# NilanEkanayake/TiTok-Video

Measured on AMD Instinct MI355X. Metric: video clips/sec encode+decode (whole node), higher is better.
Workload: dtype bf16

## Files before the change

include/titok_hip.h:

```cpp
#ifndef TITOK_HIP_H
#define TITOK_HIP_H

#include <stdint.h>

#ifdef __cplusplus
extern "C" {
#endif

#define TTV_OK 0
#define TTV_ERR_INVALID 1
#define TTV_ERR_LAUNCH 2
#define TTV_ERR_UNSUPPORTED 3

#define TTV_BF16 0
#define TTV_F32 1

#define TTV_ENCODER 0
#define TTV_DECODER 1

#define TTV_MAX_FSQ 8
#define TTV_MAX_TOKEN 64
#define TTV_MAX_CLIPS_PER_LAUNCH 64

const char* ttv_error_string(void);
// ... 112 lines not shown
int ttv_quant_v_pv8(const void* qkvg, int ld, const int32_t* cu_seqlens, int n_seqs, int total_rows, int q_heads, int kv_heads, void* image,
                    void* stream);
int ttv_attention_pv8(const void* qkvg, int ld, void* out, int ldo, const int32_t* cu_seqlens, const int32_t* qblocks, int n_qblocks,
                      int q_heads, int kv_heads, int head_dim, int flags, const void* image, void* stream);

int ttv_rmsnorm_mx(const void* in, int in_dtype, int ld_in, void* out, int out_dtype, int ld_out, const float* gain, int rows, int width,
                   float eps, float* next_rstd, void* mx_q, void* mx_s, void* stream);
int ttv_attention_mxout(const void* qkvg, int ld, void* out_q, void* out_mx, int ld_mx, const int32_t* cu_seqlens, const int32_t* qblocks,
                        int n_qblocks, int q_heads, int kv_heads, void* stream);
int ttv_linear_fp8_mx_geglu_q(const void* xq, int ldx, const void* x_mx, const float* x_row_scale, const void* wq, int ldw, const void* w_mx,
                              const float* w_row_scale, void* hq, void* hq_mx, int M, int N, int K, void* stream);

int ttv_row_rstd(const void* x, int dtype, int ldx, float* rstd, int rows, int width, float eps, void* stream);
int ttv_linear_rowscale(const void* x, int ldx, const void* w, int ldw, const float* row_scale, int epilogue, const float* rope_cs, int d_model,
                        int gqa_dim, void* y, int ldy, int M, int N, int K, int dtype, void* stream);

int ttv_patch_gather(const void* const* clips, const int32_t* clip_desc, int clip0, int n_clips, int patch_t, int patch_h,
                     int patch_w, int channels, void* patches, int ld, int dtype, int max_patches_per_clip, void* stream);
int ttv_patch_embed_norm(const void* const* clips, const int32_t* clip_desc, const int32_t* patch_rows, const int32_t* row_seq, int n_clips,
                         int patch_t, int patch_h, int patch_w, int channels, const void* w, int ldw, const void* bias,
                         const float* mask_token, const float* gain, float eps, void* x, int ldx, int rows, int width, int dtype,
                         void* stream);
int ttv_patch_scatter(const void* patches, int ld, const int32_t* clip_desc, int clip0, int n_clips, int patch_t, int patch_h,
                      int patch_w, int channels, void* const* clips, int dtype, int max_patches_per_clip, void* stream);

typedef struct ttv_tower_dims {
  int32_t kind;
  int32_t dtype;
  int32_t width;
  int32_t layers;
// ... 505 lines not shown
```

titok_video_amd/_lib.py:

```python
from __future__ import annotations

import ctypes as C
import os
import threading

import torch

from . import switches

TTV_BF16, TTV_F32 = 0, 1
TTV_ENCODER, TTV_DECODER = 0, 1
TTV_MAX_FSQ = 8
TTV_MAX_TOKEN = 64
TTV_MAX_CLIPS_PER_LAUNCH = 64
TTV_DISC_HEAD_GENERATOR, TTV_DISC_HEAD_DISCRIMINATOR = 0, 1
TTV_TAPE_STORED, TTV_TAPE_RECOMPUTE = 0, 1

DBG_NO_STORES = 1
DBG_K256_NO_PANEL_DMA = 2
DBG_MLP_NO_WEIGHT_DMA = 2
DBG_K256_NO_TILE_RELOAD = 4
DBG_MLP_NO_GEGLU = 4
DBG_K256_NO_EPILOGUE_MATH = 8
DBG_MLP_TILES8 = 8
# ... 211 lines not shown
    "ttv_layer_tail_fused": (C.c_int, [vp, C.c_int, vp, f32, vp, C.c_int, vp, C.c_int, vp, C.c_int, vp, f32, f32, C.c_int, C.c_int,
                                       C.c_int, vp, vp]),
    "ttv_mlp_fused": (C.c_int, [vp, C.c_int, vp, C.c_int, vp, C.c_int, vp, f32, f32, C.c_int, C.c_int, C.c_int, vp]),
    "ttv_fill_const_rows": (C.c_int, [vp, C.c_int, C.c_int, vp, C.c_int, C.c_int, vp, vp, f32, vp]),
    "ttv_decoder_embed": (C.c_int, [vp, C.c_int, vp, vp, vp, vp, vp, C.c_int, C.c_int, vp, C.c_int, C.c_int, f32, vp]),
    "ttv_attention": (C.c_int, [vp, C.c_int, vp, C.c_int, vp, vp, C.c_int, C.c_int, C.c_int, C.c_int, C.c_int, C.c_int, vp]),
    "ttv_attention64": (C.c_int, [vp, C.c_int, vp, C.c_int, vp, vp, C.c_int, C.c_int, C.c_int, C.c_int, C.c_int, C.c_int, vp]),
    "ttv_rmsnorm_mx": (C.c_int, [vp, C.c_int, C.c_int, vp, C.c_int, C.c_int, vp, C.c_int, C.c_int, f32, vp, vp, vp, vp]),
    "ttv_attention_pv8_bytes": (C.c_int64, [C.c_int, C.c_int, C.c_int]),
    "ttv_quant_v_pv8": (C.c_int, [vp, C.c_int, vp, C.c_int, C.c_int, C.c_int, C.c_int, vp, vp]),
    "ttv_attention_pv8": (C.c_int, [vp, C.c_int, vp, C.c_int, vp, vp, C.c_int, C.c_int, C.c_int, C.c_int, C.c_int, vp, vp]),
    "ttv_attention_mxout": (C.c_int, [vp, C.c_int, vp, vp, C.c_int, vp, vp, C.c_int, C.c_int, C.c_int, vp]),
    "ttv_linear_fp8_mx_geglu_q": (C.c_int, [vp, C.c_int, vp, vp, vp, C.c_int, vp, vp, vp, vp, C.c_int, C.c_int, C.c_int, vp]),
    "ttv_row_rstd": (C.c_int, [vp, C.c_int, C.c_int, vp, C.c_int, C.c_int, f32, vp]),
    "ttv_linear_rowscale": (C.c_int, [vp, C.c_int, vp, C.c_int, vp, C.c_int, vp, C.c_int, C.c_int, vp, C.c_int, C.c_int, C.c_int, C.c_int, C.c_int, vp]),
    "ttv_patch_gather": (C.c_int, [C.POINTER(vp), vp, C.c_int, C.c_int, C.c_int, C.c_int, C.c_int, C.c_int, vp, C.c_int,
                                   C.c_int, C.c_int, vp]),
    "ttv_patch_embed_norm": (C.c_int, [C.POINTER(vp), vp, vp, vp, C.c_int, C.c_int, C.c_int, C.c_int, C.c_int, vp, C.c_int, vp, vp, vp, f32,
                                       vp, C.c_int, C.c_int, C.c_int, C.c_int, vp]),
    "ttv_patch_scatter": (C.c_int, [vp, C.c_int, vp, C.c_int, C.c_int, C.c_int, C.c_int, C.c_int, C.c_int, C.POINTER(vp),
                                    C.c_int, C.c_int, vp]),
    "ttv_tower_workspace_bytes": (i64, [C.POINTER(TowerDims), C.POINTER(Batch)]),
    "ttv_encoder_forward": (C.c_int, [C.POINTER(TowerDims), C.POINTER(TowerWeights), C.POINTER(Batch), C.POINTER(vp),
                                      C.POINTER(FsqParams), vp, vp, vp, vp, vp, i64, vp]),
    "ttv_decoder_forward": (C.c_int, [C.POINTER(TowerDims), C.POINTER(TowerWeights), C.POINTER(Batch), vp, C.POINTER(vp),
                                      vp, i64, vp]),
    "ttv_dec_l0_const_bytes": (i64, [C.POINTER(TowerDims), C.c_int]),
    "ttv_dec_l0_const_build": (C.c_int, [C.POINTER(TowerDims), C.POINTER(TowerWeights), vp, vp, vp, vp, C.c_int, vp, i64, C.POINTER(i64), C.POINTER(i64), vp]),
    "ttv_decoder_forward_const": (C.c_int, [C.POINTER(TowerDims), C.POINTER(TowerWeights), C.POINTER(Batch), vp, C.POINTER(vp),
                                            vp, i64, C.POINTER(DecL0Const), vp]),
# ... 210 lines not shown
```

titok_video_amd/csrc/ttv_api.hip:

```cpp
#include <stdarg.h>
#include <stdio.h>
#include <stdlib.h>
#include <string.h>

#include "ttv_common.h"
#include "ttv_kernels.h"

static thread_local char g_err[512] = "";

void ttv_set_error(const char* fmt, ...) {
  va_list ap;
  va_start(ap, fmt);
  vsnprintf(g_err, sizeof(g_err), fmt, ap);
  va_end(ap);
}

int g_ttv_prof_class = 0;
bool ttv_sw_enc_latent_last() { static const bool v = ttv_env_flag("TTV_ENC_LATENT_LAST", true); return v; }
bool ttv_enc_latent_rows_only(const ttv_tower_dims* d, const ttv_batch* b) {
  return ttv_sw_enc_latent_last() && !(g_ttv_debug & TTV_DBG_ENC_ALL_ROWS) && d->kind == TTV_ENCODER && b->latent_rows && b->sum_tokens > 0 &&
         b->sum_tokens < b->total_rows;
}
bool ttv_sw_keel_f32sum() { static const bool v = ttv_env_flag("TTV_KEEL_F32SUM", false); return v; }
bool ttv_sw_fused_patch() { static const bool v = ttv_env_flag("TTV_FUSED_PATCH", true); return v; }
// ... 237 lines not shown
  const int nq = 2 * dm + 2 * g;
  const int64_t row_bytes = (int64_t)dm * dtype_bytes(dt);
  bool qkv_ready = false;
  bool rstd_valid = false;
  bool xq_valid = false;
  const bool lat_last = ttv_enc_latent_rows_only(d, b) && b->qblocks_latent && b->n_qblocks_latent > 0;
  static const bool pat_env = ttv_env_flag("TTV_DEC_PATCH_LAST", true);
  const bool pat_last = pat_env && !(g_ttv_debug & TTV_DBG_DEC_ALL_BLOCKS) && d->kind == TTV_DECODER && d->layers >= 2 && b->qblocks_patch &&
                        b->n_qblocks_patch > 0 && !split3 && !b->qblocks_paired;
  bool compacted = false;
  const bool pv8 = w->attn_pv8 != 0;
  TTV_CHECK_ARG(!pv8 || (dt == TTV_BF16 && !split3), "attn_pv8 is a bf16 inference option (not for fp32 or split-bf16 towers)");
  const LayerCtx ctx = {d, b, ws, s, split3, s3img, gen_ok, b->qblocks_paired ? TTV_ATTN_PAIRED : 0, b->qblocks_all_full ? TTV_ATTN_ALLFULL : 0,
                        ttv_sw_attn_pipe() ? TTV_ATTN_PIPE : 0, pv8};
  const bool l0_const = dec_l0_const_ok(ctx, w, l0);
  for (int i = 0; i < d->layers; ++i) {
    const ttv_layer_weights& lw = w->layers[i];
    const bool last = i == d->layers - 1;
    const bool l0c = l0_const && i == 0;
    if (dt == TTV_BF16 && dm != 256 && dm % 128 == 0 && d->inner % 128 == 0 && !ttv_sw_keel_f32sum() && lw.to_qkv_f8 && lw.to_qkv_mx && lw.w12_f8 &&
        lw.w12_mx && lw.out_proj_f8 && lw.out_proj_mx && lw.w3_f8 && lw.w3_mx &&
        !(lat_last && last)) {
      TTV_TRY(run_layer_mx(ctx, lw, i, rstd_valid, xq_valid));
      qkv_ready = false;
      continue;
    }
    xq_valid = false;
    const bool f8_qkv = rows_f8(dt, dm, lw.to_qkv_f8, lw.to_qkv_f8_scale, lw.to_qkv_mx, lw.to_qkv_pn);
    const bool f8_w12 = rows_f8(dt, dm, lw.w12_f8, lw.w12_f8_scale, lw.w12_mx, lw.w12_pn);
    if (!qkv_ready) {
      const void* w_plain = (dt == TTV_BF16 && lw.to_qkv_qs) ? lw.to_qkv_qs : lw.to_qkv;
      const PreNormW qw = {lw.pre_ln, w_plain, lw.to_qkv_pn, lw.to_qkv_f8, lw.to_qkv_f8_scale, f8_qkv};
      if (l0c) TTV_TRY(prenorm_proj(ctx, EPI_QKV_ROPE, ws.x, L, qw, nq, ws.qkv, 0, rstd_valid, l0->latent_rows / 128, (l0->latent_rows + l0->patch_rows) / 128));
      else if (lat_last && last && !f8_qkv && enc_last_qkv_skip_ok(ctx, lw))
        TTV_TRY(prenorm_proj(ctx, EPI_QKV_ROPE, ws.x, L, qw, nq, ws.qkv, 0, rstd_valid, b->tokens_per_clip / 128,
                             (b->tokens_per_clip + b->max_patches_per_clip) / 128, 2 * dm / 64));
      else TTV_TRY(prenorm_proj(ctx, EPI_QKV_ROPE, ws.x, L, qw, nq, ws.qkv, s3img ? 2 : 0, rstd_valid));
// ... 18 lines not shown
      TTV_TRY(tower_attention(ctx, q_scaled, b->qblocks, b->n_qblocks, ctx.pair | ctx.all_full | ctx.pipe));
    char* cx = ws.x;
    char* cao = ws.ao;
    int Lc = L;
    if (lat_now) {
      TTV_TRY(gather_rows(ws.x, ws.xl, b->latent_rows, b->sum_tokens, row_bytes, s));
      TTV_TRY(gather_rows(ws.ao, ws.aol, b->latent_rows, b->sum_tokens, row_bytes, s));
      cx = ws.xl; cao = ws.aol; Lc = b->sum_tokens;
      compacted = true;
    }
    static const bool use_fused_mlp = ttv_env_flag("TTV_FUSED_MLP", true);
    static const bool use_fused_qkv = ttv_env_flag("TTV_FUSED_QKV", false);
    const float alpha = keel_alpha(d, i);
    if (use_fused_mlp && ttvk_mlp_fused_supported(dt, dm, d->inner) && lw.mlp_pack) {
      MlpNextQkv nx = {};
      const bool back = use_fused_qkv && !last && lw.mlp_pack_qkv_rows == nq && nq % 64 == 0 && dm % 64 == 0 && g % 64 == 0;
      if (back) { nx.qkv = ws.qkv; nx.ld = nq; nx.rope_cs = b->rope_cs; nx.rows = nq; nx.rope_q_end = dm; nx.rope_k_begin = 2 * dm; nx.rope_k_end = 2 * dm + g; }
      TTV_TRY(ttvk_mlp_fused(cao, dm, i == 0 ? nullptr : lw.attn_post_ln, alpha, cx, dm, lw.mlp_pack, d->inner, cx, dm, i == 0 ? nullptr : lw.ffd_post_ln,
                             alpha, d->eps, Lc, back ? &nx : nullptr, s));
      qkv_ready = back;
      continue;
    }
    TTV_TRY(keel_tail(ctx, gemm_args(dt, cao, dm, lw.out_proj, dm, Lc, dm, dm, cx, dm), i, lw.attn_post_ln, gen_ok && lw.w12_pn && !f8_w12, rstd_valid));
    const PreNormW fw = {lw.ffd_norm, lw.w12, lw.w12_pn, lw.w12_f8, lw.w12_f8_scale, f8_w12};
    TTV_TRY(prenorm_proj(ctx, EPI_GEGLU, cx, Lc, fw, d->inner, ws.h, s3img, rstd_valid));
    rstd_valid = false;
    const ttv_layer_weights* nl = last ? nullptr : &w->layers[i + 1];
    const bool next_rstd = gen_ok && nl && nl->to_qkv_pn && !rows_f8(dt, dm, nl->to_qkv_f8, nl->to_qkv_f8_scale, nl->to_qkv_mx, nl->to_qkv_pn);
    TTV_TRY(keel_tail(ctx, gemm_args(dt, ws.h, d->inner, lw.w3, d->inner, Lc, dm, d->inner, cx, dm), i, lw.ffd_post_ln, next_rstd, rstd_valid));
  }
  if (compacted)
// ... 306 lines not shown
  TTV_CHECK_ARG(ldx >= width, "row_rstd: leading dim smaller than the width");
  return ttvk_row_rstd(x, dtype, ldx, rstd, rows, width, eps, (hipStream_t)stream);
}

int ttv_linear_rowscale(const void* x, int ldx, const void* w, int ldw, const float* row_scale, int epilogue, const float* rope_cs, int d_model,
                        int gqa_dim, void* y, int ldy, int M, int N, int K, int dtype, void* stream) {
  TTV_CHECK_ARG(M == 0 || (x && w && y), "linear_rowscale: null buffer");
  TTV_CHECK_ARG(epilogue >= 0 && epilogue <= 2, "linear_rowscale: epilogue 0 (store), 1 (qkv + rotary) or 2 (GEGLU)");
  GemmArgs a = gemm_args(dtype, x, ldx, w, ldw, M, N, K, y, ldy);
  if (epilogue == 1) {
    TTV_CHECK_ARG(rope_cs && N == 2 * d_model + 2 * gqa_dim && K == d_model, "linear_rowscale: qkv epilogue needs rope_cs, N = 2 d_model + 2 gqa_dim and K = d_model");
    a = gemm_rope_qk(a, rope_cs, d_model, gqa_dim);
  }
  a.row_scale = row_scale;
  return ttvk_gemm(epilogue == 0 ? EPI_STORE : epilogue == 1 ? EPI_QKV_ROPE : EPI_GEGLU, a, (hipStream_t)stream);
}

int ttv_patch_gather(const void* const* clips, const int32_t* clip_desc, int clip0, int n_clips, int patch_t, int patch_h, int patch_w,
                     int channels, void* patches, int ld, int dtype, int max_patches_per_clip, void* stream) {
  TTV_CHECK_ARG(n_clips == 0 || (clips && clip_desc && patches), "patch_gather: null buffer");
  return ttvk_patch_copy(false, (void* const*)clips, clip_desc, clip0, n_clips, patch_t, patch_h, patch_w, channels, patches, ld, dtype, max_patches_per_clip, (hipStream_t)stream);
}

int ttv_patch_embed_norm(const void* const* clips, const int32_t* clip_desc, const int32_t* patch_rows, const int32_t* row_seq, int n_clips,
                         int patch_t, int patch_h, int patch_w, int channels, const void* w, int ldw, const void* bias, const float* mask_token,
                         const float* gain, float eps, void* x, int ldx, int rows, int width, int dtype, void* stream) {
  TTV_CHECK_ARG(rows == 0 || (clips && clip_desc && patch_rows && row_seq && w && bias && mask_token && gain && x), "patch_embed_norm: null buffer");
  const int pd = channels * patch_t * patch_h * patch_w;
  if (!ttvk_patch_embed_norm_supported(dtype, width, pd, patch_w)) {
    ttv_set_error("patch_embed_norm: only bf16, width 256, patch_w 8 and a patch vector that is a multiple of 64");
// ... 411 lines not shown
```

titok_video_amd/csrc/ttv_mlp.hip:

```cpp
#include "ttv_common.h"
#include "ttv_kernels.h"

#define MLP_W12_CHUNKS 2048
#define MLP_W3_CHUNKS 1024
#define MLP_PANEL_CHUNKS (MLP_W12_CHUNKS + MLP_W3_CHUNKS)
#define MLP_WO_CHUNKS (4 * MLP_W12_CHUNKS)

struct MlpDev {
  const bf16_t* x; int ldx;
  const uint4* pack;
  const bf16_t* ao; int ldao;
  const float* front_gain;
  float front_alpha;
  bf16_t* qkv; int ldq;
  const float* rope_cs;
  int nqp, rope_q_end, rope_k_begin, rope_k_end;
  int I;
  bf16_t* y; int ldy;
  const float* post_gain;
  float alpha, eps;
  int M, n_tiles, debug;
  long long* stamps;
};

__global__ void k_mlp_pack(const bf16_t* __restrict__ w12f, const bf16_t* __restrict__ w3, const bf16_t* __restrict__ wo,
                           const bf16_t* __restrict__ wq, int nq_rows, int I, uint4* __restrict__ out) {
  const int np = I / 32;
  const int nqp = (nq_rows + 63) / 64;
  const int o = blockIdx.x * blockDim.x + threadIdx.x;
  if (o >= np * MLP_PANEL_CHUNKS + MLP_WO_CHUNKS + nqp * MLP_W12_CHUNKS) return;
  if (o >= np * MLP_PANEL_CHUNKS + MLP_WO_CHUNKS) {
    const int c = o - np * MLP_PANEL_CHUNKS - MLP_WO_CHUNKS, qp = c / MLP_W12_CHUNKS, cc = c - qp * MLP_W12_CHUNKS;
    const int r = cc >> 5, cp = cc & 31;
    const int ch = (cp & 16) | ((cp & 15) ^ (r & 15));
    int srow = qp * 64 + r;
    srow = srow < nq_rows ? srow : nq_rows - 1;
    const bf16_t* src = wq + (size_t)srow * 256 + (ch >> 2) * 32 + (ch & 3) * 4;
    const uint2 lo = *reinterpret_cast<const uint2*>(src), hi = *reinterpret_cast<const uint2*>(src + 16);
    out[o] = make_uint4(lo.x, lo.y, hi.x, hi.y);
    return;
  }
  if (o >= np * MLP_PANEL_CHUNKS) {
    const int c = o - np * MLP_PANEL_CHUNKS, wp = c / MLP_W12_CHUNKS, cc = c - wp * MLP_W12_CHUNKS;
    const int r = cc >> 5, cp = cc & 31;
    const int ch = (cp & 16) | ((cp & 15) ^ (r & 15));
    out[o] = wo ? *reinterpret_cast<const uint4*>(wo + (size_t)(wp * 64 + r) * 256 + ch * 8) : make_uint4(0, 0, 0, 0);
    return;
  }
  const int pn = o / MLP_PANEL_CHUNKS, c = o - pn * MLP_PANEL_CHUNKS;
  if (c < MLP_W12_CHUNKS) {
    const int r = c >> 5, cp = c & 31;
    const int ch = (cp & 16) | ((cp & 15) ^ (r & 15));
    const int srow = r < 32 ? pn * 32 + r : I + pn * 32 + (r - 32);
    const bf16_t* src = w12f + (size_t)srow * 256 + (ch >> 2) * 32 + (ch & 3) * 4;
// ... 24 lines not shown
                 "s_mov_b32 m0, %0"                                                                                \
                 : "=&s"(keep__)                                                                                   \
                 : "v"(lane16), "v"(lane16 + 8192u), "v"(lane16 + 16384u), "v"(lane16 + 24576u), "s"(src_), "s"(dst_) \
                 : "memory", "scc");                                                                               \
  } while (0)
#define MLP_GLDS_2(src_, dst_)                                                                                     \
  do {                                                                                                             \
    unsigned keep__;                                                                                               \
    asm volatile("s_mov_b32 %0, m0\n\t"                                                                            \
                 "s_mov_b32 m0, %4\n\ts_nop 0\n\tglobal_load_lds_dwordx4 %1, %3\n\t"                               \
                 "s_add_u32 m0, %4, 0x2000\n\ts_nop 0\n\tglobal_load_lds_dwordx4 %2, %3\n\t"                       \
                 "s_mov_b32 m0, %0"                                                                                \
                 : "=&s"(keep__)                                                                                   \
                 : "v"(lane16), "v"(lane16 + 8192u), "s"(src_), "s"(dst_)                                          \
                 : "memory", "scc");                                                                               \
  } while (0)
#ifdef MLP_STAMPS
#define MLP_STAMP()                                                                                                \
  do {                                                                                                             \
    if (p.stamps && blockIdx.x == 0 && (wave & 3) == 0 && lane == 0 && n_stamp < 64)                               \
      p.stamps[(wave >> 2) * 64 + n_stamp++] = (long long)__builtin_readcyclecounter();                            \
  } while (0)
#else
#define MLP_STAMP() do { (void)n_stamp; } while (0)
#endif

template <int TPB, int T1, int T2, bool GELU_FIRST, bool KEEL, bool FRONT, bool BACK>
__device__ __forceinline__ void mlp_wave(const MlpDev& p, uint4* l12, uint4* l3, uint4* hb, const float* gl, int tile, int wave, int lane,
                                         int P1F, int P2F, int& n_stamp) {
  constexpr int T1A = T1 > 0 ? T1 : 1, T2A = T2 > 0 ? T2 : 1;
// ... 250 lines not shown
  #pragma unroll
          for (int j = 0; j < T2; ++j) out[m][j] = __builtin_amdgcn_mfma_f32_16x16x32_bf16(w3f[m & 3], hf[j], out[m][j], 0, 0, 0);
          if (m + 4 < 16) w3f[m & 3] = __builtin_bit_cast(bf16x8, w3l[(m + 4) * 16]);
          __builtin_amdgcn_sched_group_barrier(0x008, T2A, 0);
          if (m + 4 < 16) __builtin_amdgcn_sched_group_barrier(0x100, 1, 0);
          __builtin_amdgcn_sched_barrier(0);
        }
      }
    }
    if (it >= 4 && it < 8) MLP_STAMP();
    __builtin_amdgcn_s_waitcnt(0x0F70);
    __syncthreads();
    if (it >= 4 && it < 8) MLP_STAMP();
  }
  MLP_STAMP();

  uint4* const xres = l12;
  if (FRONT) {
#pragma unroll
    for (int j = 0; j < T1; ++j)
#pragma unroll
      for (int s8 = 0; s8 < 8; ++s8) xres[((P1F + j) * 8 + s8) * 64 + lane] = __builtin_bit_cast(uint4, bfr[j][s8]);
    __syncthreads();
  }

  bf16x8 xq[T2A][8];
  float rstdq[T2A];
#pragma unroll
  for (int j = 0; j < T2; ++j) {
    const int t = tok0 + 16 * (P2F + j);
    const bool tv = t < p.M;
    const int tc = tv ? t : p.M - 1;
    const uint32_t roff = ((uint32_t)tc * (uint32_t)p.ldx + kq * 4) * 2u;
    float ss = 0.f;
#pragma unroll
    for (int s8 = 0; s8 < 8; ++s8) {
      f32x4 rv0, rv1;
      if (FRONT) {
        const bf16x8 rb = __builtin_bit_cast(bf16x8, xres[((P2F + j) * 8 + s8) * 64 + lane]);
        rv0 = (f32x4){(float)rb[0], (float)rb[1], (float)rb[2], (float)rb[3]};
        rv1 = (f32x4){(float)rb[4], (float)rb[5], (float)rb[6], (float)rb[7]};
      } else {
// ... 3 lines not shown
      out[2 * s8][j] += p.alpha * rv0;
      out[2 * s8 + 1][j] += p.alpha * rv1;
#pragma unroll
      for (int e = 0; e < 4; ++e) {
        ss = fmaf(out[2 * s8][j][e], out[2 * s8][j][e], ss);
        ss = fmaf(out[2 * s8 + 1][j][e], out[2 * s8 + 1][j][e], ss);
      }
    }
    float scale = 1.0f;
    if (KEEL) {
      ss = quad16_sum(ss);
      scale = 1.0f / sqrtf(ss * (1.0f / 256.0f) + p.eps);
    }
    const bool odd = kq & 1;
    const uint32_t yoff = ((uint32_t)tc * (uint32_t)p.ldy + (odd ? 16 + kq * 4 - 4 : kq * 4)) * 2u;
    float ssq = 0.f;
#pragma unroll
    for (int ip = 0; ip < 8; ++ip) {
      const int i0 = 2 * ip, i1 = 2 * ip + 1;
      f32x4 y0 = out[i0][j], y1 = out[i1][j];
      if (KEEL) {
        const f32x4 g0 = *reinterpret_cast<const f32x4*>(gl + i0 * 16 + kq * 4);
        const f32x4 g1 = *reinterpret_cast<const f32x4*>(gl + i1 * 16 + kq * 4);
#pragma unroll
        for (int e = 0; e < 4; ++e) { y0[e] = y0[e] * scale * g0[e]; y1[e] = y1[e] * scale * g1[e]; }
      }
      const bf16x4 q0 = {(bf16_t)y0[0], (bf16_t)y0[1], (bf16_t)y0[2], (bf16_t)y0[3]};
      const bf16x4 q1 = {(bf16_t)y1[0], (bf16_t)y1[1], (bf16_t)y1[2], (bf16_t)y1[3]};
      const uint2 p0 = __builtin_bit_cast(uint2, q0), p1 = __builtin_bit_cast(uint2, q1);
      if (BACK) {
        xq[j][ip] = __builtin_bit_cast(bf16x8, make_uint4(p0.x, p0.y, p1.x, p1.y));
#pragma unroll
        for (int e = 0; e < 4; ++e) {
          const float r0 = (float)q0[e], r1 = (float)q1[e];
          ssq = fmaf(r0, r0, ssq);
          ssq = fmaf(r1, r1, ssq);
        }
      }
      const uint4 ov = xchg16_pair(p0, p1);
      if (tv && !(p.debug & TTV_DBG_NO_STORES)) *(__attribute__((address_space(1))) u32x4_t*)(gy + yoff + ip * 64) = (u32x4_t){ov.x, ov.y, ov.z, ov.w};
    }
    if (BACK) {
      ssq = quad16_sum(ssq);
      rstdq[j] = 1.0f / sqrtf(ssq * (1.0f / 256.0f) + p.eps);
    }
  }
  MLP_STAMP();

  if (BACK) {
#define GLDS_WQ(qp_, buf_)                                                                                         \
  do {                                                                                                             \
    const uint4* src__ = p.pack + ((size_t)np * MLP_PANEL_CHUNKS + MLP_WO_CHUNKS + (qp_) * MLP_W12_CHUNKS + wave * 64); \
    const uint32_t dst__ = lds_l12 + ((buf_) * MLP_W12_CHUNKS + wave * 64) * 16;                                   \
    MLP_GLDS_4(src__, dst__);                                                                                      \
  } while (0)
    __syncthreads();
    GLDS_WQ(0, 0);
    gchar* const gq = (gchar*)p.qkv;
    gcchar* const grope = (gcchar*)p.rope_cs;
    f32x2 rc[4][T2A], rs[4][T2A];
    uint32_t qoff[T2A];
    bool qv[T2A];
#pragma unroll
    for (int j = 0; j < T2; ++j) {
      const int t = tok0 + 16 * (P2F + j);
      qv[j] = t < p.M;
      const int tc = qv[j] ? t : p.M - 1;
      qoff[j] = ((uint32_t)tc * (uint32_t)p.ldq + kq * 4) * 2u;
      gcchar* cs = grope + ((uint32_t)tc * 64u + kq * 2) * 4u;
#pragma unroll
      for (int i = 0; i < 4; ++i) {
        rc[i][j] = *(const __attribute__((address_space(1))) f32x2*)(cs + i * 32);
        rs[i][j] = *(const __attribute__((address_space(1))) f32x2*)(cs + 128 + i * 32);
      }
    }
    __builtin_amdgcn_s_waitcnt(0x0F70);
    __syncthreads();
    for (int qp = 0; qp < p.nqp; ++qp) {
      if (qp + 1 < p.nqp) GLDS_WQ(qp + 1, (qp + 1) & 1);
      const uint4* img = l12 + (qp & 1) * MLP_W12_CHUNKS;
      f32x4 qa[4][T2A];
      bf16x8 a[2][4];
#pragma unroll
      for (int i = 0; i < 4; ++i) a[0][i] = MLP_LD12(img, i, 0);
#pragma unroll
      for (int s8 = 0; s8 < 8; ++s8) {
        if (s8 + 1 < 8) {
#pragma unroll
          for (int i = 0; i < 4; ++i) a[(s8 + 1) & 1][i] = MLP_LD12(img, i, s8 + 1);
        }
#pragma unroll
        for (int i = 0; i < 4; ++i)
#pragma unroll
          for (int j = 0; j < T2; ++j)
            qa[i][j] = __builtin_amdgcn_mfma_f32_16x16x32_bf16(a[s8 & 1][i], xq[j][s8], s8 ? qa[i][j] : (f32x4){0.f, 0.f, 0.f, 0.f}, 0, 0, 0);
        if (s8 + 1 < 8) __builtin_amdgcn_sched_group_barrier(0x100, 4, 0);
        __builtin_amdgcn_sched_group_barrier(0x008, 4 * T2A, 0);
        __builtin_amdgcn_sched_barrier(0);
      }
      __builtin_amdgcn_s_waitcnt(0x0F70);
      __syncthreads();
      const int f_first = qp * 64;
      const bool rot = f_first < p.rope_q_end || (f_first >= p.rope_k_begin && f_first < p.rope_k_end);
#pragma unroll
      for (int j = 0; j < T2; ++j) {
        const bool odd = kq & 1;
        gchar* const qrow = gq + (qoff[j] - (uint32_t)(kq * 4) * 2u) + (uint32_t)(f_first + (odd ? 16 + kq * 4 - 4 : kq * 4)) * 2u;
#pragma unroll
        for (int ip = 0; ip < 2; ++ip) {
          uint2 pk[2];
#pragma unroll
          for (int u = 0; u < 2; ++u) {
            const int i = 2 * ip + u;
            f32x4 v = qa[i][j] * rstdq[j];
            if (rot)
              v = (f32x4){v[0] * rc[i][j].x - v[1] * rs[i][j].x, v[0] * rs[i][j].x + v[1] * rc[i][j].x,
                          v[2] * rc[i][j].y - v[3] * rs[i][j].y, v[2] * rs[i][j].y + v[3] * rc[i][j].y};
            const bf16x4 q = {(bf16_t)v[0], (bf16_t)v[1], (bf16_t)v[2], (bf16_t)v[3]};
            pk[u] = __builtin_bit_cast(uint2, q);
          }
          const uint4 ox = xchg16_pair(pk[0], pk[1]);
          const u32x4_t ov = {ox.x, ox.y, ox.z, ox.w};
          if (qv[j]) *(__attribute__((address_space(1))) u32x4_t*)(qrow + ip * 64) = ov;
        }
      }
    }
#undef GLDS_WQ
    MLP_STAMP();
  }
#undef GLDS_W12
#undef GLDS_W3
}

template <int TILES, bool KEEL, bool FRONT, bool BACK>
__global__ __launch_bounds__(512, 1) void k_mlp256(MlpDev p) {
  extern __shared__ __attribute__((aligned(16))) uint4 smem[];
  uint4* const l12 = smem;
  uint4* const l3 = smem + 2 * MLP_W12_CHUNKS;
  uint4* const hb = l3 + 2 * MLP_W3_CHUNKS;
  float* const gl = reinterpret_cast<float*>(hb + 2 * TILES * 64);
  if (threadIdx.x < 256) {
    gl[threadIdx.x] = p.post_gain ? p.post_gain[threadIdx.x] : 1.0f;
    gl[256 + threadIdx.x] = (FRONT && p.front_gain) ? p.front_gain[threadIdx.x] : 1.0f;
  }
  const int lane = threadIdx.x & 63;
  const int wave = __builtin_amdgcn_readfirstlane(threadIdx.x >> 6);
  int n_stamp = 0;
  const int tile = blockIdx.x;
  if constexpr (TILES == 9) {
    if (wave < 4) mlp_wave<9, 2, 0, false, KEEL, FRONT, BACK>(p, l12, l3, hb, gl, tile, wave, lane, 2 * wave, 0, n_stamp);
    else if (wave < 6) mlp_wave<9, 0, 3, false, KEEL, FRONT, BACK>(p, l12, l3, hb, gl, tile, wave, lane, 0, 3 * (wave - 4), n_stamp);
    else if (wave == 6) mlp_wave<9, 1, 1, false, KEEL, FRONT, BACK>(p, l12, l3, hb, gl, tile, wave, lane, 8, 6, n_stamp);
    else mlp_wave<9, 0, 2, false, KEEL, FRONT, BACK>(p, l12, l3, hb, gl, tile, wave, lane, 0, 7, n_stamp);
  } else {
    constexpr int NT = TILES / 4;
    constexpr int TA = NT - NT / 2;
    const int g0 = (wave & 3) * NT;
    if (wave < 4) mlp_wave<TILES, TA, NT - TA, false, KEEL, FRONT, BACK>(p, l12, l3, hb, gl, tile, wave, lane, g0, g0 + TA, n_stamp);
    else mlp_wave<TILES, NT - TA, TA, false, KEEL, FRONT, BACK>(p, l12, l3, hb, gl, tile, wave, lane, g0 + TA, g0, n_stamp);
  }
}
#undef MLP_LD12
#undef MLP_GLDS_4
#undef MLP_GLDS_2
#undef MLP_STAMP

bool ttvk_mlp_fused_supported(int dtype, int width, int inner) { return dtype == TTV_BF16 && width == 256 && inner % 32 == 0 && inner > 0; }

int64_t ttvk_mlp_pack_bytes(int inner, int next_qkv_rows) {
  if (inner <= 0 || inner % 32 != 0 || next_qkv_rows < 0) return 0;
  return ((int64_t)(inner / 32) * MLP_PANEL_CHUNKS + MLP_WO_CHUNKS + (int64_t)((next_qkv_rows + 63) / 64) * MLP_W12_CHUNKS) * 16;
}

int ttvk_mlp_pack(const void* w12_folded, const void* w3, const void* wo, const void* next_qkv_folded, int next_qkv_rows, int inner,
                  void* packed, hipStream_t s) {
  TTV_CHECK_ARG(w12_folded && w3 && packed, "mlp_pack: null buffer");
  TTV_CHECK_ARG(inner > 0 && inner % 32 == 0, "mlp_pack: inner %% 32");
  TTV_CHECK_ARG((next_qkv_folded != nullptr) == (next_qkv_rows > 0), "mlp_pack: next_qkv weight and row count must come together");
// ... 20 lines not shown
  d.qkv = nullptr; d.ldq = 0; d.rope_cs = nullptr; d.nqp = 0; d.rope_q_end = d.rope_k_begin = d.rope_k_end = 0;
  if (nq) {
    TTV_CHECK_ARG(nq->qkv && nq->rope_cs && nq->rows > 0 && nq->rows % 64 == 0 && nq->ld >= nq->rows && nq->ld % 4 == 0 &&
                      (uintptr_t)nq->qkv % 8 == 0, "mlp_fused: bad next-qkv arguments (rows %% 64, ld %% 4, 8-byte aligned)");
    TTV_CHECK_ARG(nq->rope_q_end % 64 == 0 && nq->rope_k_begin % 64 == 0 && nq->rope_k_end % 64 == 0, "mlp_fused: rotary ranges must be whole heads");
    d.qkv = (bf16_t*)nq->qkv; d.ldq = nq->ld; d.rope_cs = nq->rope_cs; d.nqp = nq->rows / 64;
    d.rope_q_end = nq->rope_q_end; d.rope_k_begin = nq->rope_k_begin; d.rope_k_end = nq->rope_k_end;
  }
  const int cus = 256;
  int tiles = 4;
  long best = -1;
  for (int c = 1; c <= 3; ++c) {
    const long cost = (long)ttv_cdiv(ttv_cdiv(M, 64 * c), cus) * (16 + 19 * c);
    if (best < 0 || cost < best) { best = cost; tiles = 4 * c; }
  }
  if (!nq && !(g_ttv_debug & TTV_DBG_MLP_PAIRS_ONLY)) {
    const long cost9 = (long)ttv_cdiv(ttv_cdiv(M, 144), cus) * (16 + 14 * 3);
    if (cost9 < best) { best = cost9; tiles = 9; }
  }
  if ((g_ttv_debug & TTV_DBG_MLP_TILES9) && !nq) tiles = 9;
  if (g_ttv_debug & TTV_DBG_MLP_TILES8) tiles = 8;
  if (g_ttv_debug & TTV_DBG_MLP_TILES4) tiles = 4;
  d.n_tiles = ttv_cdiv(M, 16 * tiles);
  const int grid = d.n_tiles;
  const size_t smem = (size_t)(2 * MLP_W12_CHUNKS + 2 * MLP_W3_CHUNKS + 2 * tiles * 64) * sizeof(uint4) + 2048;
  TtvProfScope prof(TTV_KC_GEMM_GEGLU, s);
#define LAUNCH_MLP(TILES_, KEEL_, FRONT_, BACK_)                                                                    \
  do {                                                                                                              \
    (void)hipFuncSetAttribute((const void*)k_mlp256<TILES_, KEEL_, FRONT_, BACK_>, hipFuncAttributeMaxDynamicSharedMemorySize, (int)smem); \
    hipLaunchKernelGGL((k_mlp256<TILES_, KEEL_, FRONT_, BACK_>), dim3(grid), dim3(512), smem, s, d);                \
  } while (0)
#define LAUNCH_MLP_F(TILES_, KEEL_)                                                                                 \
  do {                                                                                                              \
    if (ao && nq) LAUNCH_MLP(TILES_, KEEL_, true, true);                                                            \
    else if (ao) LAUNCH_MLP(TILES_, KEEL_, true, false);                                                            \
    else LAUNCH_MLP(TILES_, KEEL_, false, false);                                                                   \
  } while (0)
#define LAUNCH_MLP_9(KEEL_)                                                                                         \
  do {                                                                                                              \
    if (ao) LAUNCH_MLP(9, KEEL_, true, false);                                                                      \
    else LAUNCH_MLP(9, KEEL_, false, false);                                                                        \
  } while (0)
  TTV_CHECK_ARG(!nq || ao, "mlp_fused: the next-qkv part needs the out_proj front (ttv_layer_tail_fused)");
  if (post_gain) {
    if (tiles == 9) LAUNCH_MLP_9(true); else if (tiles == 12) LAUNCH_MLP_F(12, true); else if (tiles == 8) LAUNCH_MLP_F(8, true); else LAUNCH_MLP_F(4, true);
  } else {
    if (tiles == 9) LAUNCH_MLP_9(false); else if (tiles == 12) LAUNCH_MLP_F(12, false); else if (tiles == 8) LAUNCH_MLP_F(8, false); else LAUNCH_MLP_F(4, false);
  }
#undef LAUNCH_MLP_9
#undef LAUNCH_MLP_F
#undef LAUNCH_MLP
  TTV_CHECK_LAUNCH("mlp_fused");
  return TTV_OK;
}
```

Before: 32270.

## Restructure fused MLP back-end next-layer QKV projection with 32x32 MFMA and LDS handoff

The fused MLP kernel's tail, which computes the next layer's QKV projection with RMSNorm and rotary, moves into a separate device function. Output rows are handed over through the LDS xres area instead of being held in registers, and the projection now uses 32x32x16 MFMA tiles with rstd folded into the rotary coefficients. The weight prefetch is issued earlier, and the 9-tile configuration is now allowed with the back fusion. The host side limits back fusion to cases where the next layer has a pre-normed QKV and is not on the MX path, and adds a standalone prenorm QKV-rope linear entry point. The goal is lower register pressure and better MFMA use in the fused tail, at the cost of more LDS traffic and more shared memory.

```diff
diff --git a/include/titok_hip.h b/include/titok_hip.h
--- a/include/titok_hip.h
+++ b/include/titok_hip.h
@@ -150,6 +150,8 @@
 int ttv_row_rstd(const void* x, int dtype, int ldx, float* rstd, int rows, int width, float eps, void* stream);
 int ttv_linear_rowscale(const void* x, int ldx, const void* w, int ldw, const float* row_scale, int epilogue, const float* rope_cs, int d_model,
                         int gqa_dim, void* y, int ldy, int M, int N, int K, int dtype, void* stream);
+int ttv_linear_qkv_rope_prenorm(const void* x, int ldx, const void* w_folded, int ldw, void* y, int ldy, int M, int d_model, int gqa_dim,
+                                const float* rope_cs, float eps, int dtype, void* stream);
 
 int ttv_patch_gather(const void* const* clips, const int32_t* clip_desc, int clip0, int n_clips, int patch_t, int patch_h,
                      int patch_w, int channels, void* patches, int ld, int dtype, int max_patches_per_clip, void* stream);
diff --git a/titok_video_amd/_lib.py b/titok_video_amd/_lib.py
--- a/titok_video_amd/_lib.py
+++ b/titok_video_amd/_lib.py
@@ -249,6 +249,7 @@
     "ttv_linear_fp8_mx_geglu_q": (C.c_int, [vp, C.c_int, vp, vp, vp, C.c_int, vp, vp, vp, vp, C.c_int, C.c_int, C.c_int, vp]),
     "ttv_row_rstd": (C.c_int, [vp, C.c_int, C.c_int, vp, C.c_int, C.c_int, f32, vp]),
     "ttv_linear_rowscale": (C.c_int, [vp, C.c_int, vp, C.c_int, vp, C.c_int, vp, C.c_int, C.c_int, vp, C.c_int, C.c_int, C.c_int, C.c_int, C.c_int, vp]),
+    "ttv_linear_qkv_rope_prenorm": (C.c_int, [vp, C.c_int, vp, C.c_int, vp, C.c_int, C.c_int, C.c_int, C.c_int, vp, C.c_float, C.c_int, vp]),
     "ttv_patch_gather": (C.c_int, [C.POINTER(vp), vp, C.c_int, C.c_int, C.c_int, C.c_int, C.c_int, C.c_int, vp, C.c_int,
                                    C.c_int, C.c_int, vp]),
     "ttv_patch_embed_norm": (C.c_int, [C.POINTER(vp), vp, vp, vp, C.c_int, C.c_int, C.c_int, C.c_int, C.c_int, vp, C.c_int, vp, vp, vp, f32,
diff --git a/titok_video_amd/csrc/ttv_api.hip b/titok_video_amd/csrc/ttv_api.hip
--- a/titok_video_amd/csrc/ttv_api.hip
+++ b/titok_video_amd/csrc/ttv_api.hip
@@ -275,13 +275,17 @@
   const LayerCtx ctx = {d, b, ws, s, split3, s3img, gen_ok, b->qblocks_paired ? TTV_ATTN_PAIRED : 0, b->qblocks_all_full ? TTV_ATTN_ALLFULL : 0,
                         ttv_sw_attn_pipe() ? TTV_ATTN_PIPE : 0, pv8};
   const bool l0_const = dec_l0_const_ok(ctx, w, l0);
+  auto layer_mx = [&](int j) {
+    const ttv_layer_weights& m = w->layers[j];
+    return dt == TTV_BF16 && dm != 256 && dm % 128 == 0 && d->inner % 128 == 0 && !ttv_sw_keel_f32sum() && m.to_qkv_f8 && m.to_qkv_mx && m.w12_f8 &&
+           m.w12_mx && m.out_proj_f8 && m.out_proj_mx && m.w3_f8 && m.w3_mx &&
+           !(lat_last && j == d->layers - 1);
+  };
   for (int i = 0; i < d->layers; ++i) {
     const ttv_layer_weights& lw = w->layers[i];
     const bool last = i == d->layers - 1;
     const bool l0c = l0_const && i == 0;
-    if (dt == TTV_BF16 && dm != 256 && dm % 128 == 0 && d->inner % 128 == 0 && !ttv_sw_keel_f32sum() && lw.to_qkv_f8 && lw.to_qkv_mx && lw.w12_f8 &&
-        lw.w12_mx && lw.out_proj_f8 && lw.out_proj_mx && lw.w3_f8 && lw.w3_mx &&
-        !(lat_last && last)) {
+    if (layer_mx(i)) {
       TTV_TRY(run_layer_mx(ctx, lw, i, rstd_valid, xq_valid));
       qkv_ready = false;
       continue;
@@ -330,7 +334,13 @@
     const float alpha = keel_alpha(d, i);
     if (use_fused_mlp && ttvk_mlp_fused_supported(dt, dm, d->inner) && lw.mlp_pack) {
       MlpNextQkv nx = {};
-      const bool back = use_fused_qkv && !last && lw.mlp_pack_qkv_rows == nq && nq % 64 == 0 && dm % 64 == 0 && g % 64 == 0;
+      bool back = use_fused_qkv && !last && lw.mlp_pack_qkv_rows == nq && nq % 64 == 0 && dm % 64 == 0 && g % 64 == 0;
+      if (back) {
+        const ttv_layer_weights& nl = w->layers[i + 1];
+        const bool next_last = i + 1 == d->layers - 1;
+        back = nl.to_qkv_pn && !layer_mx(i + 1) && !rows_f8(dt, dm, nl.to_qkv_f8, nl.to_qkv_f8_scale, nl.to_qkv_mx, nl.to_qkv_pn) &&
+               !(lat_last && next_last && enc_last_qkv_skip_ok(ctx, nl));
+      }
       if (back) { nx.qkv = ws.qkv; nx.ld = nq; nx.rope_cs = b->rope_cs; nx.rows = nq; nx.rope_q_end = dm; nx.rope_k_begin = 2 * dm; nx.rope_k_end = 2 * dm + g; }
       TTV_TRY(ttvk_mlp_fused(cao, dm, i == 0 ? nullptr : lw.attn_post_ln, alpha, cx, dm, lw.mlp_pack, d->inner, cx, dm, i == 0 ? nullptr : lw.ffd_post_ln,
                              alpha, d->eps, Lc, back ? &nx : nullptr, s));
@@ -667,6 +677,18 @@
   }
   a.row_scale = row_scale;
   return ttvk_gemm(epilogue == 0 ? EPI_STORE : epilogue == 1 ? EPI_QKV_ROPE : EPI_GEGLU, a, (hipStream_t)stream);
+}
+
+int ttv_linear_qkv_rope_prenorm(const void* x, int ldx, const void* w_folded, int ldw, void* y, int ldy, int M, int d_model, int gqa_dim,
+                                const float* rope_cs, float eps, int dtype, void* stream) {
+  TTV_CHECK_ARG(M == 0 || (x && w_folded && y && rope_cs), "linear_qkv_rope_prenorm: null buffer");
+  if (dtype != TTV_BF16 || d_model != 256) {
+    ttv_set_error("linear_qkv_rope_prenorm: only bf16, d_model 256");
+    return TTV_ERR_UNSUPPORTED;
+  }
+  GemmArgs a = gemm_rope_qk(gemm_args(dtype, x, ldx, w_folded, ldw, M, 2 * d_model + 2 * gqa_dim, d_model, y, ldy), rope_cs, d_model, gqa_dim);
+  a.prenorm = true; a.eps = eps;
+  return ttvk_gemm(EPI_QKV_ROPE, a, (hipStream_t)stream);
 }
 
 int ttv_patch_gather(const void* const* clips, const int32_t* clip_desc, int clip0, int n_clips, int patch_t, int patch_h, int patch_w,
diff --git a/titok_video_amd/csrc/ttv_mlp.hip b/titok_video_amd/csrc/ttv_mlp.hip
--- a/titok_video_amd/csrc/ttv_mlp.hip
+++ b/titok_video_amd/csrc/ttv_mlp.hip
@@ -11,14 +11,13 @@
   const uint4* pack;
   const bf16_t* ao; int ldao;
   const float* front_gain;
-  float front_alpha;
   bf16_t* qkv; int ldq;
   const float* rope_cs;
   int nqp, rope_q_end, rope_k_begin, rope_k_end;
   int I;
   bf16_t* y; int ldy;
   const float* post_gain;
-  float alpha, eps;
+  float alpha, eps, front_alpha;
   int M, n_tiles, debug;
   long long* stamps;
 };
@@ -35,9 +34,7 @@
     const int ch = (cp & 16) | ((cp & 15) ^ (r & 15));
     int srow = qp * 64 + r;
     srow = srow < nq_rows ? srow : nq_rows - 1;
-    const bf16_t* src = wq + (size_t)srow * 256 + (ch >> 2) * 32 + (ch & 3) * 4;
-    const uint2 lo = *reinterpret_cast<const uint2*>(src), hi = *reinterpret_cast<const uint2*>(src + 16);
-    out[o] = make_uint4(lo.x, lo.y, hi.x, hi.y);
+    out[o] = *reinterpret_cast<const uint4*>(wq + (size_t)srow * 256 + ch * 8);
     return;
   }
   if (o >= np * MLP_PANEL_CHUNKS) {
@@ -92,6 +89,17 @@
                  : "=&s"(keep__)                                                                                   \
                  : "v"(lane16), "v"(lane16 + 8192u), "s"(src_), "s"(dst_)                                          \
                  : "memory", "scc");                                                                               \
+  } while (0)
+__device__ __forceinline__ const uint4* mlp_uniform_ptr(const uint4* q) {
+  const uint64_t v = (uint64_t)(uintptr_t)q;
+  const uint32_t lo = __builtin_amdgcn_readfirstlane((uint32_t)v), hi = __builtin_amdgcn_readfirstlane((uint32_t)(v >> 32));
+  return (const uint4*)(uintptr_t)(((uint64_t)hi << 32) | lo);
+}
+#define GLDS_WQ(qp_, buf_)                                                                                         \
+  do {                                                                                                             \
+    const uint4* src__ = mlp_uniform_ptr(p.pack + ((size_t)np * MLP_PANEL_CHUNKS + MLP_WO_CHUNKS + (qp_) * MLP_W12_CHUNKS + wave * 64)); \
+    const uint32_t dst__ = __builtin_amdgcn_readfirstlane(lds_stage + ((buf_) * MLP_W12_CHUNKS + wave * 64) * 16); \
+    MLP_GLDS_4(src__, dst__);                                                                                      \
   } while (0)
 #ifdef MLP_STAMPS
 #define MLP_STAMP()                                                                                                \
@@ -372,6 +380,10 @@
     if (it >= 4 && it < 8) MLP_STAMP();
   }
   MLP_STAMP();
+  if (BACK && TPB != 12) {
+    const uint32_t lds_stage = lds_l12 + TPB * 8192;
+    GLDS_WQ(0, 0);
+  }
 
   uint4* const xres = l12;
   if (FRONT) {
@@ -382,8 +394,7 @@
     __syncthreads();
   }
 
-  bf16x8 xq[T2A][8];
-  float rstdq[T2A];
+  static_assert(!BACK || FRONT, "the fused back hands its rows over in the xres area of the fused front");
 #pragma unroll
   for (int j = 0; j < T2; ++j) {
     const int t = tok0 + 16 * (P2F + j);
@@ -417,7 +428,6 @@
     }
     const bool odd = kq & 1;
     const uint32_t yoff = ((uint32_t)tc * (uint32_t)p.ldy + (odd ? 16 + kq * 4 - 4 : kq * 4)) * 2u;
-    float ssq = 0.f;
 #pragma unroll
     for (int ip = 0; ip < 8; ++ip) {
       const int i0 = 2 * ip, i1 = 2 * ip + 1;
@@ -431,108 +441,169 @@
       const bf16x4 q0 = {(bf16_t)y0[0], (bf16_t)y0[1], (bf16_t)y0[2], (bf16_t)y0[3]};
       const bf16x4 q1 = {(bf16_t)y1[0], (bf16_t)y1[1], (bf16_t)y1[2], (bf16_t)y1[3]};
       const uint2 p0 = __builtin_bit_cast(uint2, q0), p1 = __builtin_bit_cast(uint2, q1);
-      if (BACK) {
-        xq[j][ip] = __builtin_bit_cast(bf16x8, make_uint4(p0.x, p0.y, p1.x, p1.y));
-#pragma unroll
-        for (int e = 0; e < 4; ++e) {
-          const float r0 = (float)q0[e], r1 = (float)q1[e];
-          ssq = fmaf(r0, r0, ssq);
-          ssq = fmaf(r1, r1, ssq);
-        }
-      }
+      if (BACK) xres[((P2F + j) * 8 + ip) * 64 + lane] = make_uint4(p0.x, p0.y, p1.x, p1.y);
       const uint4 ov = xchg16_pair(p0, p1);
       if (tv && !(p.debug & TTV_DBG_NO_STORES)) *(__attribute__((address_space(1))) u32x4_t*)(gy + yoff + ip * 64) = (u32x4_t){ov.x, ov.y, ov.z, ov.w};
     }
-    if (BACK) {
-      ssq = quad16_sum(ssq);
-      rstdq[j] = 1.0f / sqrtf(ssq * (1.0f / 256.0f) + p.eps);
-    }
   }
   MLP_STAMP();
-
-  if (BACK) {
-#define GLDS_WQ(qp_, buf_)                                                                                         \
-  do {                                                                                                             \
-    const uint4* src__ = p.pack + ((size_t)np * MLP_PANEL_CHUNKS + MLP_WO_CHUNKS + (qp_) * MLP_W12_CHUNKS + wave * 64); \
-    const uint32_t dst__ = lds_l12 + ((buf_) * MLP_W12_CHUNKS + wave * 64) * 16;                                   \
-    MLP_GLDS_4(src__, dst__);                                                                                      \
-  } while (0)
-    __syncthreads();
-    GLDS_WQ(0, 0);
-    gchar* const gq = (gchar*)p.qkv;
-    gcchar* const grope = (gcchar*)p.rope_cs;
-    f32x2 rc[4][T2A], rs[4][T2A];
-    uint32_t qoff[T2A];
-    bool qv[T2A];
-#pragma unroll
-    for (int j = 0; j < T2; ++j) {
-      const int t = tok0 + 16 * (P2F + j);
-      qv[j] = t < p.M;
-      const int tc = qv[j] ? t : p.M - 1;
-      qoff[j] = ((uint32_t)tc * (uint32_t)p.ldq + kq * 4) * 2u;
-      gcchar* cs = grope + ((uint32_t)tc * 64u + kq * 2) * 4u;
-#pragma unroll
-      for (int i = 0; i < 4; ++i) {
-        rc[i][j] = *(const __attribute__((address_space(1))) f32x2*)(cs + i * 32);
-        rs[i][j] = *(const __attribute__((address_space(1))) f32x2*)(cs + 128 + i * 32);
-      }
-    }
-    __builtin_amdgcn_s_waitcnt(0x0F70);
-    __syncthreads();
-    for (int qp = 0; qp < p.nqp; ++qp) {
-      if (qp + 1 < p.nqp) GLDS_WQ(qp + 1, (qp + 1) & 1);
-      const uint4* img = l12 + (qp & 1) * MLP_W12_CHUNKS;
-      f32x4 qa[4][T2A];
-      bf16x8 a[2][4];
-#pragma unroll
-      for (int i = 0; i < 4; ++i) a[0][i] = MLP_LD12(img, i, 0);
-#pragma unroll
-      for (int s8 = 0; s8 < 8; ++s8) {
-        if (s8 + 1 < 8) {
-#pragma unroll
-          for (int i = 0; i < 4; ++i) a[(s8 + 1) & 1][i] = MLP_LD12(img, i, s8 + 1);
-        }
-#pragma unroll
-        for (int i = 0; i < 4; ++i)
-#pragma unroll
-          for (int j = 0; j < T2; ++j)
-            qa[i][j] = __builtin_amdgcn_mfma_f32_16x16x32_bf16(a[s8 & 1][i], xq[j][s8], s8 ? qa[i][j] : (f32x4){0.f, 0.f, 0.f, 0.f}, 0, 0, 0);
-        if (s8 + 1 < 8) __builtin_amdgcn_sched_group_barrier(0x100, 4, 0);
-        __builtin_amdgcn_sched_group_barrier(0x008, 4 * T2A, 0);
-        __builtin_amdgcn_sched_barrier(0);
-      }
-      __builtin_amdgcn_s_waitcnt(0x0F70);
-      __syncthreads();
-      const int f_first = qp * 64;
-      const bool rot = f_first < p.rope_q_end || (f_first >= p.rope_k_begin && f_first < p.rope_k_end);
-#pragma unroll
-      for (int j = 0; j < T2; ++j) {
-        const bool odd = kq & 1;
-        gchar* const qrow = gq + (qoff[j] - (uint32_t)(kq * 4) * 2u) + (uint32_t)(f_first + (odd ? 16 + kq * 4 - 4 : kq * 4)) * 2u;
-#pragma unroll
-        for (int ip = 0; ip < 2; ++ip) {
-          uint2 pk[2];
-#pragma unroll
-          for (int u = 0; u < 2; ++u) {
-            const int i = 2 * ip + u;
-            f32x4 v = qa[i][j] * rstdq[j];
-            if (rot)
-              v = (f32x4){v[0] * rc[i][j].x - v[1] * rs[i][j].x, v[0] * rs[i][j].x + v[1] * rc[i][j].x,
-                          v[2] * rc[i][j].y - v[3] * rs[i][j].y, v[2] * rs[i][j].y + v[3] * rc[i][j].y};
-            const bf16x4 q = {(bf16_t)v[0], (bf16_t)v[1], (bf16_t)v[2], (bf16_t)v[3]};
-            pk[u] = __builtin_bit_cast(uint2, q);
-          }
-          const uint4 ox = xchg16_pair(pk[0], pk[1]);
-          const u32x4_t ov = {ox.x, ox.y, ox.z, ox.w};
-          if (qv[j]) *(__attribute__((address_space(1))) u32x4_t*)(qrow + ip * 64) = ov;
-        }
-      }
-    }
-#undef GLDS_WQ
-    MLP_STAMP();
-  }
 #undef GLDS_W12
 #undef GLDS_W3
+}
+
+
+template <bool ROT>
+__device__ __forceinline__ void mlp_back_store(const f32x16& acc, const float2 (&kc)[4][2], float rstd,
+                                               __attribute__((address_space(1))) char* ydst, bool st) {
+  u32x2_t pk[2];
+#pragma unroll
+  for (int g = 0; g < 4; ++g) {
+    const float a0 = acc[4 * g], a1 = acc[4 * g + 1], a2 = acc[4 * g + 2], a3 = acc[4 * g + 3];
+    float o[4];
+    if (ROT) {
+      const float2 k0 = kc[g][0], k1 = kc[g][1];
+      o[0] = a0 * k0.x - a1 * k0.y; o[1] = a0 * k0.y + a1 * k0.x;
+      o[2] = a2 * k1.x - a3 * k1.y; o[3] = a2 * k1.y + a3 * k1.x;
+    } else {
+      o[0] = a0 * rstd; o[1] = a1 * rstd; o[2] = a2 * rstd; o[3] = a3 * rstd;
+    }
+    const bf16x4 b = {(bf16_t)o[0], (bf16_t)o[1], (bf16_t)o[2], (bf16_t)o[3]};
+    pk[g & 1] = __builtin_bit_cast(u32x2_t, b);
+    if (g & 1) {
+      const auto sx = __builtin_amdgcn_permlane32_swap(pk[0].x, pk[1].x, false, false);
+      const auto sy = __builtin_amdgcn_permlane32_swap(pk[0].y, pk[1].y, false, false);
+      const u32x4_t ov = {sx[0], sy[0], sx[1], sy[1]};
+      if (st) *(__attribute__((address_space(1))) u32x4_t*)(ydst + (g >> 1) * 32) = ov;
+    }
+  }
+}
+
+template <int TILES>
+__device__ __forceinline__ void mlp_back(const MlpDev& p, uint4* smem, int tile, int wave, int lane, int& n_stamp) {
+  constexpr int NP = (TILES + 1) / 2;
+  constexpr int NS = NP > 4 ? 2 : 1;
+  const int r = lane & 31, h = lane >> 5, r15 = r & 15;
+  const int np = p.I / 32;
+  const uint32_t lane16 = lane * 16;
+  const char* const xt = reinterpret_cast<const char*>(smem);
+  uint4* const stage = smem + TILES * 512;
+  const uint32_t lds_stage = (uint32_t)(uintptr_t)(__attribute__((address_space(3))) void*)stage;
+  typedef __attribute__((address_space(1))) char gchar;
+  typedef __attribute__((address_space(1))) const char gcchar;
+  gchar* const gq = (gchar*)p.qkv;
+  gcchar* const grope = (gcchar*)p.rope_cs;
+
+  __syncthreads();
+  if (TILES == 12) GLDS_WQ(0, 0);
+
+  bf16x8 bfr[NS][16];
+  float2 kc[NS][4][2];
+  float rstd[NS];
+  uint32_t yoff[NS];
+  uint32_t aoff[NS];
+  bool qv[NS], have[NS], full[NS];
+#pragma unroll
+  for (int s = 0; s < NS; ++s) {
+#ifdef MLP_BACK_NINTH_ROBIN
+    const int pr = s == 0 ? (wave & 3) : TILES == 9 ? 4 : 4 + (wave >> 1);
+#else
+    const int pr = s == 0 ? (wave & 3) : 4 + (wave >> 1);
+#endif
+    const int half = s == 0 ? (wave >> 2) : (wave & 1);
+    const int t0 = tile * (16 * TILES) + 32 * pr;
+    const int ntok = 16 * TILES - 32 * pr < 32 ? 16 * TILES - 32 * pr : 32;
+    have[s] = (s == 0 || wave < 4) && pr < NP && t0 < p.M;
+    full[s] = t0 + ntok <= p.M;
+    qv[s] = false; yoff[s] = 0; aoff[s] = 0; rstd[s] = 1.f;
+    if (have[s]) {
+      const int rr = r < ntok ? r : r - 16;
+      qv[s] = r < ntok && t0 + r < p.M;
+      const int tc = t0 + rr < p.M ? t0 + rr : p.M - 1;
+      yoff[s] = ((uint32_t)tc * (uint32_t)p.ldq + 32 * half + 8 * h) * 2u;
+      aoff[s] = (uint32_t)((32 * half + r) * 32 + (h ^ r15)) * 16u;
+      gcchar* cs = grope + ((uint32_t)tc * 64u + 16 * half + 2 * h) * 4u;
+#pragma unroll
+      for (int g = 0; g < 4; ++g) {
+        const f32x2 cc = *(const __attribute__((address_space(1))) f32x2*)(cs + g * 16);
+        const f32x2 sn = *(const __attribute__((address_space(1))) f32x2*)(cs + 128 + g * 16);
+        kc[s][g][0] = make_float2(cc.x, sn.x);
+        kc[s][g][1] = make_float2(cc.y, sn.y);
+      }
+      const char* xl = xt + ((2 * pr + (rr >> 4)) * 512 + 2 * h * 16 + (rr & 15)) * 16;
+      float ss0 = 0.f, ss1 = 0.f;
+#pragma unroll
+      for (int ks = 0; ks < 16; ++ks) {
+        const u32x2_t lo = *reinterpret_cast<const u32x2_t*>(xl + (ks >> 1) * 1024 + (ks & 1) * 8);
+        const u32x2_t hi = *reinterpret_cast<const u32x2_t*>(xl + (ks >> 1) * 1024 + 256 + (ks & 1) * 8);
+        const bf16x8 v = __builtin_bit_cast(bf16x8, (u32x4_t){lo.x, lo.y, hi.x, hi.y});
+        bfr[s][ks] = v;
+        ss0 = __builtin_amdgcn_fdot2_f32_bf16((bf16x2){v[0], v[1]}, (bf16x2){v[0], v[1]}, ss0, false);
+        ss1 = __builtin_amdgcn_fdot2_f32_bf16((bf16x2){v[2], v[3]}, (bf16x2){v[2], v[3]}, ss1, false);
+        ss0 = __builtin_amdgcn_fdot2_f32_bf16((bf16x2){v[4], v[5]}, (bf16x2){v[4], v[5]}, ss0, false);
+        ss1 = __builtin_amdgcn_fdot2_f32_bf16((bf16x2){v[6], v[7]}, (bf16x2){v[6], v[7]}, ss1, false);
+      }
+      float ss = ss0 + ss1;
+      ss = pair32_sum(ss);
+      rstd[s] = 1.0f / sqrtf(ss * (1.0f / 256.0f) + p.eps);
+#pragma unroll
+      for (int g = 0; g < 4; ++g)
+#pragma unroll
+        for (int e = 0; e < 2; ++e) kc[s][g][e] = make_float2(kc[s][g][e].x * rstd[s], kc[s][g][e].y * rstd[s]);
+    }
+  }
+  const bool count_ok = !(p.debug & TTV_DBG_NO_STORES);
+  const f32x16 zero16 = {0.f, 0.f, 0.f, 0.f, 0.f, 0.f, 0.f, 0.f, 0.f, 0.f, 0.f, 0.f, 0.f, 0.f, 0.f, 0.f};
+  asm volatile("s_waitcnt vmcnt(0)" ::: "memory");
+  __syncthreads();
+  MLP_STAMP();
+  for (int qp = 0; qp < p.nqp; ++qp) {
+    if (qp + 1 < p.nqp) GLDS_WQ(qp + 1, (qp + 1) & 1);
+    const char* const img = reinterpret_cast<const char*>(stage + (qp & 1) * MLP_W12_CHUNKS);
+    const int f_first = qp * 64;
+    const bool rot = f_first < p.rope_q_end || (f_first >= p.rope_k_begin && f_first < p.rope_k_end);
+    int n_stores = 0;
+    bool counted = count_ok;
+#pragma unroll
+    for (int s = 0; s < NS; ++s) {
+      bool mine = have[s];
+#ifdef MLP_BACK_NINTH_ROBIN
+      if (TILES == 9 && s == 1) mine = mine && (qp & 1) == (wave >> 1);
+#else
+      if (TILES == 9 && s == 1) mine = mine && wave < 2;
+#endif
+      if (!mine) continue;
+#define BACK_AFRAG(ks_) (*reinterpret_cast<const bf16x8*>(img + (aoff[s] ^ (uint32_t)(((ks_) & 7) << 5)) + (((ks_) >> 3) & 1) * 256))
+      f32x16 acc;
+      bf16x8 af[8];
+#pragma unroll
+      for (int i = 0; i < 8; ++i) af[i] = BACK_AFRAG(i);
+      __builtin_amdgcn_sched_barrier(0);
+#pragma unroll
+      for (int ks = 0; ks < 16; ++ks) {
+        acc = __builtin_amdgcn_mfma_f32_32x32x16_bf16(af[ks & 7], bfr[s][ks], ks ? acc : zero16, 0, 0, 0);
+        if (ks + 8 < 16) af[ks & 7] = BACK_AFRAG(ks + 8);
+        __builtin_amdgcn_sched_group_barrier(0x008, 1, 0);
+        if (ks + 8 < 16) __builtin_amdgcn_sched_group_barrier(0x100, 1, 0);
+        __builtin_amdgcn_sched_barrier(0);
+      }
+#undef BACK_AFRAG
+      gchar* const ydst = gq + yoff[s] + (uint32_t)f_first * 2u;
+      const bool st = qv[s] && count_ok;
+      if (rot) mlp_back_store<true>(acc, kc[s], rstd[s], ydst, st);
+      else mlp_back_store<false>(acc, kc[s], rstd[s], ydst, st);
+      n_stores += 2;
+      counted = counted && full[s];
+    }
+    MLP_STAMP();
+    if (qp + 1 < p.nqp) {
+      if (counted && n_stores == 4) asm volatile("s_waitcnt vmcnt(4)" ::: "memory");
+      else if (counted && n_stores == 2) asm volatile("s_waitcnt vmcnt(2)" ::: "memory");
+      else asm volatile("s_waitcnt vmcnt(0)" ::: "memory");
+      __builtin_amdgcn_s_barrier();
+      asm volatile("" ::: "memory");
+    }
+    MLP_STAMP();
+  }
 }
 
 template <int TILES, bool KEEL, bool FRONT, bool BACK>
@@ -562,9 +633,11 @@
     if (wave < 4) mlp_wave<TILES, TA, NT - TA, false, KEEL, FRONT, BACK>(p, l12, l3, hb, gl, tile, wave, lane, g0, g0 + TA, n_stamp);
     else mlp_wave<TILES, NT - TA, TA, false, KEEL, FRONT, BACK>(p, l12, l3, hb, gl, tile, wave, lane, g0 + TA, g0, n_stamp);
   }
+  if constexpr (BACK) mlp_back<TILES>(p, smem, tile, wave, lane, n_stamp);
 }
 #undef MLP_LD12
 #undef MLP_GLDS_4
+#undef GLDS_WQ
 #undef MLP_GLDS_2
 #undef MLP_STAMP
 
@@ -615,16 +688,20 @@
     const long cost = (long)ttv_cdiv(ttv_cdiv(M, 64 * c), cus) * (16 + 19 * c);
     if (best < 0 || cost < best) { best = cost; tiles = 4 * c; }
   }
-  if (!nq && !(g_ttv_debug & TTV_DBG_MLP_PAIRS_ONLY)) {
+  if (!(g_ttv_debug & TTV_DBG_MLP_PAIRS_ONLY)) {
     const long cost9 = (long)ttv_cdiv(ttv_cdiv(M, 144), cus) * (16 + 14 * 3);
     if (cost9 < best) { best = cost9; tiles = 9; }
   }
-  if ((g_ttv_debug & TTV_DBG_MLP_TILES9) && !nq) tiles = 9;
+  if (g_ttv_debug & TTV_DBG_MLP_TILES9) tiles = 9;
   if (g_ttv_debug & TTV_DBG_MLP_TILES8) tiles = 8;
   if (g_ttv_debug & TTV_DBG_MLP_TILES4) tiles = 4;
   d.n_tiles = ttv_cdiv(M, 16 * tiles);
   const int grid = d.n_tiles;
-  const size_t smem = (size_t)(2 * MLP_W12_CHUNKS + 2 * MLP_W3_CHUNKS + 2 * tiles * 64) * sizeof(uint4) + 2048;
+  size_t smem = (size_t)(2 * MLP_W12_CHUNKS + 2 * MLP_W3_CHUNKS + 2 * tiles * 64) * sizeof(uint4) + 2048;
+  if (nq) {
+    const size_t back = (size_t)(tiles * 512 + 2 * MLP_W12_CHUNKS) * sizeof(uint4);
+    smem = back > smem ? back : smem;
+  }
   TtvProfScope prof(TTV_KC_GEMM_GEGLU, s);
 #define LAUNCH_MLP(TILES_, KEEL_, FRONT_, BACK_)                                                                    \
   do {                                                                                                              \
@@ -639,7 +716,8 @@
   } while (0)
 #define LAUNCH_MLP_9(KEEL_)                                                                                         \
   do {                                                                                                              \
-    if (ao) LAUNCH_MLP(9, KEEL_, true, false);                                                                      \
+    if (ao && nq) LAUNCH_MLP(9, KEEL_, true, true);                                                                 \
+    else if (ao) LAUNCH_MLP(9, KEEL_, true, false);                                                                 \
     else LAUNCH_MLP(9, KEEL_, false, false);                                                                        \
   } while (0)
   TTV_CHECK_ARG(!nq || ao, "mlp_fused: the next-qkv part needs the out_proj front (ttv_layer_tail_fused)");
```

Result: no change. 32250, median of 2 (-0.1%).
